# shaofeifei11/SSDR-AL

Hardware: AMD Instinct MI355X
Metric: Mpoints/s subsample→KNN→RandLA-Net→FPS-GCN select, S3DIS 40960-pt tiles (higher is better)
Workload: dtype bf16x3: split-bf16 MFMA operands (hi*hi + lo*hi + hi*lo), fp32 accumulate, fp32 activations and non-matrix arithmetic

## Files before the change

### ssdr-al_amd/csrc/block_prims.hpp

```cpp
#pragma once
#include "ssdr_internal.hpp"
#include <cfloat>

namespace ssdr {

constexpr int BS = 256;
constexpr int U = 4;
constexpr int CHUNK = BS * U;

#ifndef HIPEMU
template <class Op>
__device__ __forceinline__ unsigned wave_reduce_u32(unsigned x, Op op) {
    x = op(x, (unsigned)__builtin_amdgcn_update_dpp((int)x, (int)x, 0xB1, 0xf, 0xf, true));
    x = op(x, (unsigned)__builtin_amdgcn_update_dpp((int)x, (int)x, 0x4E, 0xf, 0xf, true));
    x = op(x, (unsigned)__builtin_amdgcn_update_dpp((int)x, (int)x, 0x141, 0xf, 0xf, true));
    x = op(x, (unsigned)__builtin_amdgcn_update_dpp((int)x, (int)x, 0x140, 0xf, 0xf, true));
    auto r = __builtin_amdgcn_permlane16_swap(x, x, false, false);
    x = op(r[0], r[1]);
    r = __builtin_amdgcn_permlane32_swap(x, x, false, false);
    return op(r[0], r[1]);
}
__device__ __forceinline__ float wave_min(float v) {
    return __uint_as_float(wave_reduce_u32(__float_as_uint(v), [](unsigned a, unsigned b) { return __float_as_uint(fminf(__uint_as_float(a), __uint_as_float(b))); }));
}
// ... 28 lines not shown
        const int lin = tile * gx + bx, xcd = lin & 7, j = lin >> 3;
        tile = xcd + 8 * (j / gx); bx = j % gx;
    }
}

__device__ __forceinline__ void wave_sync() {
#ifndef HIPEMU
    __builtin_amdgcn_fence(__ATOMIC_RELEASE, "workgroup");
    __builtin_amdgcn_wave_barrier();
    __builtin_amdgcn_fence(__ATOMIC_ACQUIRE, "workgroup");
#else
    (void)__shfl(0, 0);
#endif
}

template <int NT = BS>
__device__ inline void block_minmax3(float (&mn)[3], float (&mx)[3], float* s ) {
    const int lane = threadIdx.x & 63, wid = threadIdx.x >> 6;
#pragma unroll
    for (int d = 0; d < 3; ++d) {
        float a = wave_min(mn[d]), b = wave_max(mx[d]);
        if (lane == 0) { s[wid * 6 + d] = a; s[wid * 6 + 3 + d] = b; }
    }
    __syncthreads();
#pragma unroll
    for (int d = 0; d < 3; ++d) {
        float a = s[d], b = s[3 + d];
#pragma unroll
        for (int w = 1; w < NT / 64; ++w) { a = fminf(a, s[w * 6 + d]); b = fmaxf(b, s[w * 6 + 3 + d]); }
        mn[d] = a; mx[d] = b;
// ... 49 lines not shown
```

### ssdr-al_amd/csrc/frontend.hip

```cpp
#include "ssdr_internal.hpp"
#include "block_prims.hpp"
#include "voxel_label.hpp"
#include "subsample_types.hpp"

namespace ssdr {
namespace {

constexpr int FE_NBMAX = 16384;
constexpr int FE_CH = 32768;
constexpr int FE_NT = 1024;
constexpr int FE_PPT = 12, FE_SNT = 1024;
#ifndef FE_PAIR_STORES
#define FE_PAIR_STORES 1
#endif
constexpr int FE_LR = 64;
constexpr int FE_VMAX = 1024;
#ifndef FE_RNT_OPT
#define FE_RNT_OPT 128
#endif
constexpr int FE_RNT = FE_RNT_OPT;
#ifndef FE_WALK_OPT
#define FE_WALK_OPT 4
#endif
constexpr int FE_WALK = FE_WALK_OPT;
constexpr int FE_CAP = 1024;
constexpr int FE_RPT = FE_CAP / FE_RNT;
constexpr int FE_SLICES = 62;
constexpr int FE_ROWCAP = FE_LR * FE_NBMAX;

struct FeGeom {
    float org[3]; float dl;
    int nx, ny, nz, sx;
    int nbx, nby, nbz, nb;
    int ok, n, pad0, pad1;
};
struct FeItem { unsigned base, n, rb, sx; float org[3]; float dl; };

struct FeTab { int nr; int chunks_max; int ovf_cap; int n_total; int off[RADIX_MAX_SEG + 1]; };

__device__ __forceinline__ bool fe_voxel(const FeGeom& g, float x, float y, float z, int& ix, int& iy, int& iz) {
    const float fx = floorf((x - g.org[0]) / g.dl), fy = floorf((y - g.org[1]) / g.dl), fz = floorf((z - g.org[2]) / g.dl);
    const bool ok = fx >= 0.f && fx < (float)g.nx && fy >= 0.f && fy < (float)g.ny && fz >= 0.f && fz < (float)g.nz;
    ix = (int)fx; iy = (int)fy; iz = (int)fz;
    return ok;
}
__device__ __forceinline__ int fe_bucket(const FeGeom& g, int ix, int iy, int iz) { return (ix >> g.sx) + g.nbx * ((iy >> 3) + g.nby * (iz >> 3)); }
__device__ __forceinline__ int fe_vid(const FeItem& it, float x, float y, float z) {
    const int ix = (int)floorf((x - it.org[0]) / it.dl), iy = (int)floorf((y - it.org[1]) / it.dl), iz = (int)floorf((z - it.org[2]) / it.dl);
    return (ix & ((1 << it.sx) - 1)) | (((iy & 7) | ((iz & 7) << 3)) << it.sx);
}

__global__ __launch_bounds__(BS) void fe_minmax_partial(FeTab t, const float* __restrict__ P, float* partial) {
    const int r = blockIdx.y;
    gs_minmax_partial_body(P + 3 * (size_t)t.off[r], t.off[r + 1] - t.off[r], partial + (size_t)r * PB * 6);
}

__global__ void fe_rcp_init(float* rcp) { const int k = blockIdx.x * blockDim.x + threadIdx.x; if (k <= FE_CAP) rcp[k] = k ? (float)(1.0 / (double)k) : 0.f; }

__global__ __launch_bounds__(BS) void fe_params(FeTab t, const float* partial, float dl, GsParams* prm, FeGeom* geom, int* counters) {
    __shared__ float s_mm[(BS / 64) * 6];
    const int r = blockIdx.x;
    float mn[3] = {FLT_MAX, FLT_MAX, FLT_MAX}, mx[3] = {-FLT_MAX, -FLT_MAX, -FLT_MAX};
    for (int i = threadIdx.x; i < PB; i += BS) {
#pragma unroll
        for (int d = 0; d < 3; ++d) { mn[d] = fminf(mn[d], partial[((size_t)r * PB + i) * 6 + d]); mx[d] = fmaxf(mx[d], partial[((size_t)r * PB + i) * 6 + 3 + d]); }
    }
    block_minmax3(mn, mx, s_mm);
    if (threadIdx.x == 0) {
        if (r == 0) { for (int i = 0; i < 8; ++i) counters[i] = 0; }
        GsParams p; FeGeom g;
        const float inv = 1 / dl;
        float nd[3];
#pragma unroll
        for (int d = 0; d < 3; ++d) { g.org[d] = floorf(mn[d] * inv) * dl; p.org[d] = g.org[d]; nd[d] = floorf((mx[d] - g.org[d]) / dl) + 1.f; }
        g.dl = dl; p.dl = dl;
        bool ok = nd[0] >= 1.f && nd[1] >= 1.f && nd[2] >= 1.f && nd[0] < 65536.f && nd[1] < 1.0e6f && nd[2] < 1.0e6f;
#pragma unroll
        for (int d = 0; d < 3; ++d) ok = ok && floorf((mn[d] - g.org[d]) / dl) >= 0.f;
        g.nx = ok ? (int)nd[0] : 1; g.ny = ok ? (int)nd[1] : 1; g.nz = ok ? (int)nd[2] : 1;
        p.nx = (unsigned long long)g.nx; p.ny = (unsigned long long)g.ny; p.m = 0; p.status = 0; p.key_and = 0ull; p.key_or = ~0ull;
        g.nby = (g.ny + 7) >> 3; g.nbz = (g.nz + 7) >> 3;
        g.sx = 3; g.nbx = (g.nx + 7) >> 3;
        if ((long long)g.nbx * g.nby * g.nbz > FE_NBMAX) { g.sx = 4; g.nbx = (g.nx + 15) >> 4; }
        if ((long long)g.nbx * g.nby * g.nbz > FE_NBMAX) ok = false;
        g.nb = ok ? g.nbx * g.nby * g.nbz : 0;
        g.ok = ok ? 1 : 0; g.n = t.off[r + 1] - t.off[r]; g.pad0 = g.pad1 = 0;
        if (!ok) p.status = 2;
        prm[r] = p; geom[r] = g;
    }
}

__global__ __launch_bounds__(FE_NT) void fe_count(FeTab t, const float* __restrict__ P, const FeGeom* __restrict__ geom, GsParams* prm, unsigned* cntm) {
    __shared__ unsigned s_h[FE_NBMAX];
    const int r = blockIdx.y, c = blockIdx.x, tid = threadIdx.x;
    const FeGeom g = geom[r];
    if (!g.ok || c * FE_CH >= g.n) return;
    for (int b = tid; b < g.nb; b += FE_NT) s_h[b] = 0u;
    __syncthreads();
    const float* Pr = P + 3 * (size_t)t.off[r];
    const int hi = min(g.n, (c + 1) * FE_CH);
    bool bad = false;
    for (int i = c * FE_CH + tid; i < hi; i += FE_NT) {
        int ix, iy, iz;
        if (fe_voxel(g, Pr[3 * (size_t)i], Pr[3 * (size_t)i + 1], Pr[3 * (size_t)i + 2], ix, iy, iz)) atomicAdd(&s_h[fe_bucket(g, ix, iy, iz)], 1u);
// ... 7 lines not shown

__device__ __forceinline__ unsigned long long fe_block_scan(unsigned long long v, unsigned long long* s_w, int nt, unsigned long long& total) {
    const int tid = threadIdx.x, lane = tid & 63, wid = tid >> 6;
    unsigned long long incl = v;
#pragma unroll
    for (int o = 1; o < 64; o <<= 1) { const unsigned long long y = __shfl_up(incl, o); if (lane >= o) incl += y; }
    if (lane == 63) s_w[wid] = incl;
    __syncthreads();
    unsigned long long wbase = 0, tot = 0;
    for (int w = 0; w < nt / 64; ++w) { const unsigned long long cw = s_w[w]; if (w < wid) wbase += cw; tot += cw; }
    __syncthreads();
    total = tot;
    return wbase + incl - v;
}

__global__ __launch_bounds__(BS) void fe_colscan(FeTab t, const FeGeom* __restrict__ geom, unsigned* cntm, unsigned* tot) {
    const int r = blockIdx.y, b = blockIdx.x * BS + threadIdx.x;
    const FeGeom g = geom[r];
    if (!g.ok || b >= g.nb) return;
    const int nchunk = (g.n + FE_CH - 1) / FE_CH;
    unsigned* cm = cntm + (size_t)r * t.chunks_max * FE_NBMAX + b;
    unsigned run = 0;
    for (int c0 = 0; c0 < nchunk; c0 += 8) {
        unsigned v[8];
#pragma unroll
        for (int u = 0; u < 8; ++u) v[u] = c0 + u < nchunk ? cm[(size_t)(c0 + u) * FE_NBMAX] : 0u;
#pragma unroll
        for (int u = 0; u < 8; ++u) if (c0 + u < nchunk) { cm[(size_t)(c0 + u) * FE_NBMAX] = run; run += v[u]; }
    }
    tot[(size_t)r * FE_NBMAX + b] = run;
}

__global__ __launch_bounds__(FE_NT) void fe_bscan(FeTab t, const FeGeom* __restrict__ geom, const unsigned* __restrict__ tot, unsigned* boff, FeItem* items, int* counters) {
    __shared__ unsigned long long s_w[FE_NT / 64];
    __shared__ unsigned s_base;
    const int r = blockIdx.x, tid = threadIdx.x;
    const FeGeom g = geom[r];
    unsigned* bo = boff + (size_t)r * (FE_NBMAX + 1);
    if (!g.ok) { if (tid == 0) bo[0] = 0u; return; }
    unsigned long long carry = 0;
    for (int b0 = 0; b0 < g.nb; b0 += FE_NT) {
        const int b = b0 + tid;
        const unsigned n = b < g.nb ? tot[(size_t)r * FE_NBMAX + b] : 0u;
        unsigned long long total;
        const unsigned long long ex = fe_block_scan(((unsigned long long)n << 20) | (n ? 1ull : 0ull), s_w, FE_NT, total);
        const unsigned start = (unsigned)((carry + ex) >> 20);
        if (b < g.nb) bo[b] = start;
        const unsigned nne = (unsigned)(total & 0xfffffull);
        if (tid == 0) s_base = nne ? (unsigned)atomicAdd(&counters[0], (int)nne) : 0u;
        __syncthreads();
        if (n) {
            FeItem it; it.base = (unsigned)t.off[r] + start; it.n = n; it.rb = ((unsigned)r << 16) | (unsigned)b; it.sx = (unsigned)g.sx;
            it.org[0] = g.org[0]; it.org[1] = g.org[1]; it.org[2] = g.org[2]; it.dl = g.dl;
            items[s_base + (unsigned)(ex & 0xfffffull)] = it;
        }
        carry += total & ~0xfffffull;
        __syncthreads();
    }
// ... 342 lines not shown
                FE_STAMP(2);
                if (ns > 0) fe_reduce_voxels<FD, LD, IMG>(L, a, &prm->status, L.orank[v0], L.orank[v1], s0, rows, R);
                FE_STAMP(3);
            }
            if (tid == 0) { a.nocc[tb] = (unsigned)nocc; a.trow[tb] = (fast && IMG) ? it.base : 0x80000000u | L.ovf; }
            for (int l = tid; l < FE_LR; l += FE_RNT) a.lrc[tb * FE_LR + l] = (unsigned char)(L.orank[(l + 1) << it.sx] - L.orank[l << it.sx]);
        }
        __syncthreads();
        FE_STAMP(4);
    }
#ifdef SSDR_FE_STAMPS
    if (tid == 0) for (int k = 0; k < 5; ++k) atomicAdd(reinterpret_cast<unsigned long long*>(a.counters) + 8 + k, t_acc[k]);
#endif
}

__global__ __launch_bounds__(BS) void fe_rowpre(const FeGeom* __restrict__ geom, const unsigned* __restrict__ boff, const unsigned char* __restrict__ lrc,
                                                unsigned short* pre, unsigned* rowcnt) {
    const int r = blockIdx.y;
    const FeGeom g = geom[r];
    if (!g.ok) return;
    const int ry = g.nby * 8, prows = ry * g.nbz * 8;
    const unsigned* bo = boff + (size_t)r * (FE_NBMAX + 1);
    for (int pr = blockIdx.x * BS + threadIdx.x; pr < prows; pr += gridDim.x * BS) {
        const int iy = pr % ry, iz = pr / ry;
        const int l = (iy & 7) | ((iz & 7) << 3);
        const int b0 = g.nbx * ((iy >> 3) + g.nby * (iz >> 3));
        unsigned run = 0;
        for (int bx = 0; bx < g.nbx; ++bx) {
            const int b = b0 + bx;
            if (bo[b + 1] != bo[b]) {
                const size_t at = ((size_t)r * FE_NBMAX + b) * FE_LR + l;
                pre[at] = (unsigned short)run;
                run += lrc[at];
            }
        }
        rowcnt[(size_t)r * FE_ROWCAP + pr] = run;
    }
}

__global__ __launch_bounds__(FE_NT) void fe_rowscan(const FeGeom* __restrict__ geom, unsigned* rowcnt, GsParams* prm, long long* out_m) {
    __shared__ unsigned long long s_w[FE_NT / 64];
    const int r = blockIdx.x, tid = threadIdx.x;
    const FeGeom g = geom[r];
    if (!g.ok) { if (tid == 0) { prm[r].m = 0; if (out_m) out_m[r] = 0; } return; }
    const int prows = g.nby * 8 * g.nbz * 8;
    unsigned* rc = rowcnt + (size_t)r * FE_ROWCAP;
    unsigned long long carry = 0;
    for (int p0 = 0; p0 < prows; p0 += FE_NT) {
        const int p = p0 + tid;
        const unsigned v = p < prows ? rc[p] : 0u;
        unsigned long long total;
        const unsigned long long ex = fe_block_scan((unsigned long long)v, s_w, FE_NT, total);
        if (p < prows) rc[p] = (unsigned)(carry + ex);
        carry += total;
    }
    if (tid == 0) { prm[r].m = (int)carry; if (out_m) out_m[r] = (long long)carry; }
}

struct FeMoveArgs {
    FeTab t; const FeGeom* geom; const FeItem* items; const int* counters; const uint4* rec; const unsigned* nocc; const unsigned* trow;
    const unsigned char* lrc; const unsigned short* pre; const unsigned* rowbase; int fdim, ldim; float* out_p; float* out_f; int* out_c;
};
template <int FD, int LD>
__global__ __launch_bounds__(BS) void fe_move(FeMoveArgs a) {
    const int fdim = FD >= 0 ? FD : a.fdim, ldim = LD >= 0 ? LD : a.ldim;
// ... 58 lines not shown
    FeTab t; t.nr = (int)nr;
    int maxn = 0;
    for (size_t r = 0; r < nr; ++r) {
        const long n = (long)(room_off[r + 1] - room_off[r]);
        if (n <= 0 || room_off[r + 1] > 0x3fffffff) { set_error("grid_subsample_batch: every cloud needs >= 1 point"); return n <= 0 ? SSDR_ERR_EMPTY : SSDR_ERR_INVALID; }
        t.off[r] = (int)room_off[r]; maxn = std::max(maxn, (int)n);
    }
    t.off[nr] = (int)room_off[nr];
    t.n_total = (int)room_off[nr];
    t.chunks_max = (maxn + FE_CH - 1) / FE_CH;
    static const bool fe_image = [] { const char* e = getenv("SSDR_FE_IMAGE"); return e && e[0] == '1'; }();
    static const int fe_wgs = [] { const char* e = getenv("SSDR_FE_WGS"); return e ? atoi(e) : 0; }();
    static const int fe_pad = [] { const char* e = getenv("SSDR_FE_PADLDS"); return e ? atoi(e) : 0; }();
    t.ovf_cap = fe_image ? std::max(65536, t.n_total / 8) : t.n_total;
    const unsigned R = (unsigned)nr;
    SSDR_TRY(S.partial.reserve(24 * (size_t)PB * nr)); SSDR_TRY(S.geom.reserve(sizeof(FeGeom) * nr)); SSDR_TRY(S.counters.reserve(256));
    SSDR_TRY(S.cntm.reserve(4 * (size_t)FE_NBMAX * t.chunks_max * nr)); SSDR_TRY(S.tot.reserve(4 * (size_t)FE_NBMAX * nr)); SSDR_TRY(S.boff.reserve(4 * (size_t)(FE_NBMAX + 1) * nr));
    SSDR_TRY(S.items.reserve(sizeof(FeItem) * (size_t)FE_NBMAX * nr)); SSDR_TRY(S.nocc.reserve(4 * (size_t)FE_NBMAX * nr)); SSDR_TRY(S.trow.reserve(4 * (size_t)FE_NBMAX * nr));
    SSDR_TRY(S.lrc.reserve((size_t)FE_NBMAX * FE_LR * nr)); SSDR_TRY(S.pre.reserve(2 * (size_t)FE_NBMAX * FE_LR * nr));
    SSDR_TRY(S.rowcnt.reserve(4 * (size_t)FE_ROWCAP * nr));
    SSDR_TRY(S.rec.reserve(32 * ((size_t)t.n_total + t.ovf_cap) + 64));
    if (!S.rcp_ready) {
        SSDR_TRY(S.rcp.reserve(4 * (FE_CAP + 1)));
        hipLaunchKernelGGL(fe_rcp_init, dim3((FE_CAP + 256) / 256), dim3(256), 0, s, S.rcp.as<float>());
        S.rcp_ready = true;
    }
    FeGeom* geom = S.geom.as<FeGeom>(); int* counters = S.counters.as<int>(); FeItem* items = S.items.as<FeItem>();
    {
    ProfScope prof("fe_bbox_count_scan", s, 0.0);
    hipLaunchKernelGGL(fe_minmax_partial, dim3(PB, R), dim3(BS), 0, s, t, d_p, S.partial.as<float>());
    hipLaunchKernelGGL(fe_params, dim3(R), dim3(BS), 0, s, t, S.partial.as<float>(), dl, prm, geom, counters);
    hipLaunchKernelGGL(fe_count, dim3(t.chunks_max, R), dim3(FE_NT), 0, s, t, d_p, geom, prm, S.cntm.as<unsigned>());
    hipLaunchKernelGGL(fe_colscan, dim3(FE_NBMAX / BS, R), dim3(BS), 0, s, t, geom, S.cntm.as<unsigned>(), S.tot.as<unsigned>());
    hipLaunchKernelGGL(fe_bscan, dim3(R), dim3(FE_NT), 0, s, t, geom, S.tot.as<unsigned>(), S.boff.as<unsigned>(), items, counters);
    }
    {
    ProfScope prof("fe_scatter", s, (double)(12 + 4 * (fdim + ldim)) * (double)t.n_total);
    if (fdim == 3 && ldim == 1)
        hipLaunchKernelGGL((fe_scatter<3, 1>), dim3(t.chunks_max, R), dim3(FE_SNT), 0, s, t, d_p, d_f, (int)fdim, (const int*)d_c, (int)ldim, geom, S.cntm.as<unsigned>(), S.boff.as<unsigned>(),
                           S.rec.as<uint4>());
    else
        hipLaunchKernelGGL((fe_scatter<-1, -1>), dim3(t.chunks_max, R), dim3(FE_SNT), 0, s, t, d_p, d_f, (int)fdim, (const int*)d_c, (int)ldim, geom, S.cntm.as<unsigned>(), S.boff.as<unsigned>(),
                           S.rec.as<uint4>());
    }
    FeRedArgs ra; ra.t = t; ra.items = items; ra.prm = prm; ra.counters = counters; ra.rcp = S.rcp.as<float>(); ra.rec = S.rec.as<uint4>();
    ra.nocc = S.nocc.as<unsigned>(); ra.trow = S.trow.as<unsigned>(); ra.lrc = S.lrc.as<unsigned char>(); ra.fdim = (int)fdim; ra.ldim = (int)ldim;
    {
    ProfScope prof("fe_reduce", s, 0.0);
    if (!fe_image) {
        const long cap = std::max<long>((long)ctx().num_cu * 16, (long)t.n_total / 64);
        const int g = (int)std::min<long>((long)ctx().num_cu * (fe_wgs > 0 ? fe_wgs : 128), fe_wgs > 0 ? (1L << 30) : cap);
        if (fdim == 3 && ldim == 1) hipLaunchKernelGGL((fe_reduce<3, 1, false>), dim3(g), dim3(FE_RNT), (size_t)fe_pad, s, ra);
        else hipLaunchKernelGGL((fe_reduce<-1, -1, false>), dim3(g), dim3(FE_RNT), (size_t)fe_pad, s, ra);
    } else if (fdim == 3 && ldim == 1) hipLaunchKernelGGL((fe_reduce<3, 1, true>), dim3(ctx().num_cu * (fe_wgs > 0 ? fe_wgs : 3)), dim3(FE_RNT), 0, s, ra);
    else hipLaunchKernelGGL((fe_reduce<-1, -1, true>), dim3(ctx().num_cu * (fe_wgs > 0 ? fe_wgs : 3)), dim3(FE_RNT), 0, s, ra);
    }
    ProfScope prof_move("fe_rows_move", s, 0.0);
    hipLaunchKernelGGL(fe_rowpre, dim3(256, R), dim3(BS), 0, s, geom, S.boff.as<unsigned>(), S.lrc.as<unsigned char>(), S.pre.as<unsigned short>(), S.rowcnt.as<unsigned>());
    hipLaunchKernelGGL(fe_rowscan, dim3(R), dim3(FE_NT), 0, s, geom, S.rowcnt.as<unsigned>(), prm, (long long*)d_om);
    FeMoveArgs ma; ma.t = t; ma.geom = geom; ma.items = items; ma.counters = counters; ma.rec = S.rec.as<uint4>(); ma.nocc = S.nocc.as<unsigned>();
    ma.trow = S.trow.as<unsigned>(); ma.lrc = S.lrc.as<unsigned char>(); ma.pre = S.pre.as<unsigned short>(); ma.rowbase = S.rowcnt.as<unsigned>(); ma.fdim = (int)fdim; ma.ldim = (int)ldim;
    ma.out_p = d_op; ma.out_f = d_of; ma.out_c = d_oc;
    static const int mv_wgs = [] { const char* e = getenv("SSDR_FE_MOVE_WGS"); return e ? atoi(e) : 32; }();
    if (fdim == 3 && ldim == 1) hipLaunchKernelGGL((fe_move<3, 1>), dim3(ctx().num_cu * mv_wgs), dim3(BS), 0, s, ma);
    else hipLaunchKernelGGL((fe_move<-1, -1>), dim3(ctx().num_cu * mv_wgs), dim3(BS), 0, s, ma);
    SSDR_HIP(hipGetLastError());
#ifdef SSDR_FE_STAMPS
    {
        SSDR_HIP(hipStreamSynchronize(s));
        unsigned long long h[8]; int hc[8];
        SSDR_HIP(hipMemcpy(hc, counters, sizeof(hc), hipMemcpyDeviceToHost));
        SSDR_HIP(hipMemcpy(h, reinterpret_cast<unsigned long long*>(counters) + 8, sizeof(h), hipMemcpyDeviceToHost));
        fprintf(stderr, "fe_reduce: %d items, %d overflow rows; clock ticks per phase (sum over workgroups): load+hist %llu, segments %llu, rank %llu, voxels %llu, tail %llu\n",
                hc[0], hc[3], h[0], h[1], h[2], h[3], h[4]);
// ... 8 lines not shown
```

### ssdr-al_amd/csrc/tile.hip

```cpp
#include "ssdr_internal.hpp"
#include "block_prims.hpp"
#include "tile_body.hpp"
#include <map>
#include <vector>

namespace ssdr {
namespace {

__device__ __forceinline__ void tile_keys_body(const float* __restrict__ pts, const long long* __restrict__ d_m, int n_host, float cx, float cy, float cz,
                                                 uint64_t* keys, uint32_t* vals, int* d_count) {
    const int m = (int)min((long long)n_host, *d_m);
    if (blockIdx.x == 0 && threadIdx.x == 0) *d_count = m;
    for (int i = blockIdx.x * 256 + threadIdx.x; i < m; i += gridDim.x * 256) {
        const float dx = pts[3 * (size_t)i] - cx, dy = pts[3 * (size_t)i + 1] - cy, dz = pts[3 * (size_t)i + 2] - cz;
        const float d = (dx * dx + dy * dy) + dz * dz;
        if (vals) { keys[i] = (uint64_t)__float_as_uint(d); vals[i] = (uint32_t)i; }
        else keys[i] = ((uint64_t)__float_as_uint(d) << 32) | (uint64_t)(uint32_t)i;
    }
}


__global__ __launch_bounds__(256) void tile_keys(const float* __restrict__ pts, const long long* __restrict__ d_m, int n_host, float cx, float cy, float cz, uint64_t* keys, uint32_t* vals, int* d_count) { tile_keys_body(pts, d_m, n_host, cx, cy, cz, keys, vals, d_count); }
__global__ __launch_bounds__(256) void tile_padmap(const int* __restrict__ d_count, int num_points, const int* __restrict__ perm, int* padmap) { __shared__ unsigned s_part[256]; tile_padmap_body(*d_count, num_points, perm, padmap, s_part); }
__global__ __launch_bounds__(256) void tile_gather(const float* __restrict__ pts, const float* __restrict__ colors, int cdim, const uint32_t* __restrict__ sorted, const int* __restrict__ d_count, const int* __restrict__ perm, const float* __restrict__ dup_u, int num_points, float cx, float cy, float cz, float color_scale, float* out_xyz, float* out_feat, int* out_idx, const int* __restrict__ padmap) { tile_gather_body(pts, colors, cdim, sorted, d_count, perm, dup_u, num_points, cx, cy, cz, color_scale, out_xyz, out_feat, out_idx, padmap); }
// ... 5 lines not shown
    tile_keys_body(pts + 3 * (size_t)t.off[r], d_m + r, t.off[r + 1] - t.off[r], t.cx[r], t.cy[r], t.cz[r], keys + t.toff[r], vals ? vals + t.toff[r] : nullptr, d_count + r);
}
__global__ __launch_bounds__(256) void tile_gather_b(TileTab t, const float* __restrict__ pts, const float* __restrict__ colors, int cdim, const uint32_t* __restrict__ sorted,
                                                     const int* __restrict__ d_count, const int* __restrict__ perm, const float* __restrict__ dup_u, int num_points,
                                                     float color_scale, float* out_xyz, float* out_feat, int* out_idx, int stride,
                                                     const int* __restrict__ labels, int* out_lab, const int* __restrict__ padmap) {
    int bx, r; xcd_tile_map(bx, r);
    const size_t o = (size_t)t.off[r], q = (size_t)r * num_points;
    tile_gather_body(pts + 3 * o, colors ? colors + o * cdim : nullptr, cdim, sorted + (size_t)t.toff[r] * stride, d_count + r, perm + q, dup_u + q, num_points, t.cx[r], t.cy[r], t.cz[r],
                     color_scale, out_xyz + 3 * q, out_feat ? out_feat + q * (3 + cdim) : nullptr, out_idx ? out_idx + q : nullptr, padmap + q, stride, bx,
                     labels ? labels + o : nullptr, out_lab ? out_lab + q : nullptr);
}

constexpr int TS_BITS = 14, TS_BINS = 1 << TS_BITS, TS_SHIFT = 31 - TS_BITS;

__global__ __launch_bounds__(256) void tile_hist_b(TileTab t, const float* __restrict__ pts, const long long* __restrict__ d_m, unsigned* hist, int* d_count) {
    __shared__ unsigned s_h[TS_BINS];
    const int r = blockIdx.y, n_host = t.off[r + 1] - t.off[r];
    const int m = (int)min((long long)n_host, d_m[r]);
    if (blockIdx.x == 0 && threadIdx.x == 0) d_count[r] = m;
    if ((int)blockIdx.x * 256 >= m) return;
    for (int b = threadIdx.x; b < TS_BINS; b += 256) s_h[b] = 0u;
    __syncthreads();
    const float* P = pts + 3 * (size_t)t.off[r];
    for (int i = blockIdx.x * 256 + threadIdx.x; i < m; i += gridDim.x * 256)
        atomicAdd(&s_h[__float_as_uint(tile_dist(P, i, t.cx[r], t.cy[r], t.cz[r])) >> TS_SHIFT], 1u);
    __syncthreads();
    for (int b = threadIdx.x; b < TS_BINS; b += 256) if (s_h[b]) atomicAdd(&hist[(size_t)r * TS_BINS + b], s_h[b]);
}
constexpr int TS_RCAP = 4096, TS_RSTEP = 1024;
__global__ __launch_bounds__(256) void tile_thresh_b(TileTab t, unsigned* hist, const int* __restrict__ d_count, int num_points, unsigned* thr, int* d_cand, unsigned* rstart, unsigned* rcur, int rstride,
                                                     const int* __restrict__ perm, int* padmap) {
    __shared__ unsigned s_h[TS_BINS + TS_BINS / 32];
    __shared__ unsigned s_part[256];
    __shared__ unsigned s_T;
    const int r = blockIdx.x, tid = threadIdx.x;
    unsigned* h = hist + (size_t)r * TS_BINS;
    unsigned* RS = rstart + (size_t)r * rstride;
    constexpr int PER = TS_BINS / 256;
    auto at = [](int b) { return b + (b >> 5); };
    const unsigned want = (unsigned)min(num_points, d_count[r]);
    for (int b = tid; b < TS_BINS; b += 256) s_h[at(b)] = h[b];
    for (int k = tid; k < rstride; k += 256) { RS[k] = 0xffffffffu; rcur[(size_t)r * rstride + k] = 0u; }
    __syncthreads();
    unsigned tot = 0;
    for (int k = 0; k < PER; ++k) tot += s_h[at(tid * PER + k)];
    s_part[tid] = tot;
    __syncthreads();
    unsigned incl = tot;
    for (int o = 1; o < 256; o <<= 1) {
        const unsigned y = tid >= o ? s_part[tid - o] : 0u;
        __syncthreads();
        incl += y; s_part[tid] = incl;
        __syncthreads();
    }
    const unsigned before = incl - tot;
    if (want > 0 && before < want && incl >= want) {
// ... 5 lines not shown
    __syncthreads();
    const unsigned T = s_T;
    unsigned pos = before, ncand = 0;
    for (int k = 0; k < PER; ++k) {
        const int b = tid * PER + k;
        const unsigned cb = s_h[at(b)];
        if ((unsigned)b <= T) {
            s_h[at(b)] = pos;
            if (cb) atomicMin(&RS[pos / TS_RSTEP], pos);
            pos += cb; ncand = pos;
        } else s_h[at(b)] = 0u;
    }
    if ((unsigned)(tid * PER) <= T && (unsigned)(tid * PER + PER - 1) >= T) { thr[r] = T; d_cand[r] = (int)ncand; }
    __syncthreads();
    for (int b = tid; b < TS_BINS; b += 256) h[b] = s_h[at(b)];
    tile_padmap_body(d_count[r], num_points, perm + (size_t)r * num_points, padmap + (size_t)r * num_points, s_part);
}
constexpr int TS_CPT = 12;
constexpr int TS_RMAX = 2048;
__global__ __launch_bounds__(256) void tile_compact_b(TileTab t, const float* __restrict__ pts, const int* __restrict__ d_count, const unsigned* __restrict__ thr,
                                                      const unsigned* __restrict__ hist, const unsigned* __restrict__ rstart, unsigned* rcur, int rstride, uint64_t* keys) {
    __shared__ unsigned s_cnt[TS_RMAX], s_base[TS_RMAX];
    const int r = blockIdx.y, m = d_count[r], tid = threadIdx.x;
    const float* P = pts + 3 * (size_t)t.off[r];
    const unsigned T = thr[r];
    const unsigned* h = hist + (size_t)r * TS_BINS;
    const unsigned* RS = rstart + (size_t)r * rstride;
    unsigned* RC = rcur + (size_t)r * rstride;
    uint64_t* K = keys + t.toff[r];
    for (int i0 = blockIdx.x * 256 * TS_CPT; i0 < m; i0 += gridDim.x * 256 * TS_CPT) {
        for (int k = tid; k < rstride; k += 256) s_cnt[k] = 0u;
// ... 18 lines not shown
        __syncthreads();
    }
}
__global__ __launch_bounds__(256) void tile_compact_bins_b(TileTab t, const float* __restrict__ pts, const int* __restrict__ d_count, const unsigned* __restrict__ thr, unsigned* hist, uint64_t* keys) {
    const int r = blockIdx.y, m = d_count[r];
    const float* P = pts + 3 * (size_t)t.off[r];
    const unsigned T = thr[r];
    unsigned* cur = hist + (size_t)r * TS_BINS;
    uint64_t* K = keys + t.toff[r];
    for (int i = blockIdx.x * 256 + threadIdx.x; i < m; i += gridDim.x * 256) {
        const unsigned bits = __float_as_uint(tile_dist(P, i, t.cx[r], t.cy[r], t.cz[r]));
        const unsigned b = bits >> TS_SHIFT;
        if (b <= T) K[atomicAdd(&cur[b], 1u)] = ((uint64_t)bits << 32) | (uint64_t)(uint32_t)i;
    }
}
__global__ __launch_bounds__(256) void tile_clear_b(unsigned* hist) {
    for (int b = blockIdx.x * 256 + threadIdx.x; b < TS_BINS; b += gridDim.x * 256) hist[(size_t)blockIdx.y * TS_BINS + b] = 0u;
}
__global__ __launch_bounds__(256) void tile_binsort_b(TileTab t, const unsigned* __restrict__ rstart, int rstride, const int* __restrict__ d_cand, uint64_t* keys) {
    __shared__ uint64_t s_k[TS_RCAP];
    const int r = blockIdx.y, tid = threadIdx.x;
    const unsigned* RS = rstart + (size_t)r * rstride;
    uint64_t* K = keys + t.toff[r];
    const unsigned cand = (unsigned)d_cand[r];
    const int nk = (int)((cand + TS_RSTEP - 1) / TS_RSTEP);
    for (int q = blockIdx.x; q < nk; q += gridDim.x) {
        const unsigned s0 = RS[q];
        if (s0 == 0xffffffffu) continue;
        unsigned e0 = cand;
        for (int q2 = q + 1; q2 < nk; ++q2) if (RS[q2] != 0xffffffffu) { e0 = RS[q2]; break; }
        const unsigned n = e0 - s0;
        if (n <= 1) continue;
        unsigned N = 2; while (N < n) N <<= 1;
        const bool lds = n <= (unsigned)TS_RCAP;
        uint64_t* A = lds ? s_k : K + s0;
        if (N <= 2048u && N >= 16u) {
// ... 139 lines not shown
    if (d_out_feat && color_dim > 0 && !d_colors) { set_error("tile_select_batch: colors missing"); return SSDR_ERR_INVALID; }
    SSDR_TRY(ensure_init());
    hipStream_t s = pick_stream(stream); TileState& T = tst(s);
    TileTab t; t.nr = (int)num_clouds;
    int toff = 0, maxn = 0; std::vector<int> n_host(num_clouds);
    for (size_t r = 0; r < num_clouds; ++r) {
        const long n = (long)(cloud_offsets[r + 1] - cloud_offsets[r]);
        if (n <= 0 || cloud_offsets[r + 1] > 0x3fffffff) { set_error("tile_select_batch: bad cloud offsets"); return SSDR_ERR_INVALID; }
        t.off[r] = (int)cloud_offsets[r]; t.toff[r] = toff; n_host[r] = (int)n; maxn = std::max(maxn, (int)n);
        t.cx[r] = centers[3 * r]; t.cy[r] = centers[3 * r + 1]; t.cz[r] = centers[3 * r + 2];
        toff += ((int)n + RADIX_TILE - 1) / RADIX_TILE * RADIX_TILE;
    }
    t.off[num_clouds] = (int)cloud_offsets[num_clouds]; t.toff[num_clouds] = toff;
    SSDR_TRY(T.keys.reserve(8 * (size_t)toff + 16)); SSDR_TRY(T.count.reserve(4 * num_clouds + 16));
    const int rstride = (maxn + TS_RSTEP - 1) / TS_RSTEP + 1;
    SSDR_TRY(T.hist.reserve(4 * (size_t)TS_BINS * RADIX_MAX_SEG)); SSDR_TRY(T.thr.reserve(4 * RADIX_MAX_SEG)); SSDR_TRY(T.cand.reserve(4 * RADIX_MAX_SEG));
    SSDR_TRY(T.rstart.reserve(4 * (size_t)rstride * num_clouds)); SSDR_TRY(T.rcur.reserve(4 * (size_t)rstride * num_clouds));
    SSDR_TRY(T.padmap.reserve(4 * num_clouds * num_points));
    if (!T.hist_clear) { SSDR_HIP(hipMemsetAsync(T.hist.p, 0, 4 * (size_t)TS_BINS * RADIX_MAX_SEG, s)); T.hist_clear = true; }
    const unsigned R = (unsigned)num_clouds;
    const int g = std::max(1, std::min((maxn + 255) / 256, 64));
    ProfScope prof("tile_select", s, (12.0 + 4.0 * (12 + 4 * (d_out_feat ? color_dim + 3 : 0))) * 0.0 + 40.0 * (double)num_clouds * (double)num_points);
    hipLaunchKernelGGL(tile_hist_b, dim3(g, R), dim3(256), 0, s, t, d_points, (const long long*)d_m, T.hist.as<unsigned>(), T.count.as<int>());
    hipLaunchKernelGGL(tile_thresh_b, dim3(R), dim3(256), 0, s, t, T.hist.as<unsigned>(), T.count.as<int>(), (int)num_points, T.thr.as<unsigned>(), T.cand.as<int>(), T.rstart.as<unsigned>(), T.rcur.as<unsigned>(), rstride,
                       d_perm, T.padmap.as<int>());
    if (rstride <= TS_RMAX)
        hipLaunchKernelGGL(tile_compact_b, dim3(std::max(1, std::min((maxn + 256 * TS_CPT - 1) / (256 * TS_CPT), 256)), R), dim3(256), 0, s, t, d_points, T.count.as<int>(), T.thr.as<unsigned>(),
                           T.hist.as<unsigned>(), T.rstart.as<unsigned>(), T.rcur.as<unsigned>(), rstride, T.keys.as<uint64_t>());
    else hipLaunchKernelGGL(tile_compact_bins_b, dim3(g, R), dim3(256), 0, s, t, d_points, T.count.as<int>(), T.thr.as<unsigned>(), T.hist.as<unsigned>(), T.keys.as<uint64_t>());
    hipLaunchKernelGGL(tile_clear_b, dim3(8, R), dim3(256), 0, s, T.hist.as<unsigned>());
    hipLaunchKernelGGL(tile_binsort_b, dim3(std::min(rstride, 64), R), dim3(256), 0, s, t, T.rstart.as<unsigned>(), rstride, T.cand.as<int>(), T.keys.as<uint64_t>());
    const int g2 = (int)std::max<size_t>(1, std::min<size_t>((num_points + 255) / 256, 256));
    hipLaunchKernelGGL(tile_gather_b, dim3(g2, R), dim3(256), 0, s, t, d_points, d_colors, d_colors ? color_dim : 0, reinterpret_cast<const uint32_t*>(T.keys.as<uint64_t>()), T.count.as<int>(),
                       d_perm, d_dup_u, (int)num_points, color_scale, d_out_xyz, d_out_feat, d_out_idx, 2, d_labels, d_out_labels, T.padmap.as<int>());
    SSDR_HIP(hipGetLastError());
    return SSDR_OK;
}
```

Before: 205.1.

## Fuse dependent frontend and tile-select kernel pairs via last-workgroup tickets

Merges several producer/consumer kernel pairs (minmax→params, colscan→bscan, rowpre→rowscan, hist→thresh) into single launches. The last workgroup to finish, detected with a per-cloud atomic ticket counter, runs the serial tail. The histogram clear is folded into binsort. This removes kernel launches and inter-kernel gaps in small, latency-bound stages. In exchange it adds atomic tickets and fences, and the tail now runs in only one workgroup, with changed block sizes for colscan and rowpre. The tickets reset themselves, so correctness depends on every workgroup reaching the ticket.

After: 155.7. -24.1%, worse.

```diff
diff --git a/ssdr-al_amd/csrc/block_prims.hpp b/ssdr-al_amd/csrc/block_prims.hpp
--- a/ssdr-al_amd/csrc/block_prims.hpp
+++ b/ssdr-al_amd/csrc/block_prims.hpp
@@ -66,6 +66,29 @@
 #endif
 }
 
+template <class T>
+__device__ __forceinline__ T dev_load(const T* p) {
+#ifndef HIPEMU
+    return __hip_atomic_load(p, __ATOMIC_RELAXED, __HIP_MEMORY_SCOPE_AGENT);
+#else
+    T v; __atomic_load(p, &v, __ATOMIC_RELAXED); return v;
+#endif
+}
+__device__ __forceinline__ bool last_workgroup(int* ticket, int expected) {
+    __shared__ int s_last;
+    __threadfence();
+    __syncthreads();
+    if (threadIdx.x == 0) {
+        const int last = atomicAdd(ticket, 1) == expected - 1 ? 1 : 0;
+        if (last) atomicExch(ticket, 0);
+        s_last = last;
+    }
+    __syncthreads();
+    const bool last = s_last != 0;
+    if (last) __threadfence();
+    return last;
+}
+
 template <int NT = BS>
 __device__ inline void block_minmax3(float (&mn)[3], float (&mx)[3], float* s ) {
     const int lane = threadIdx.x & 63, wid = threadIdx.x >> 6;
diff --git a/ssdr-al_amd/csrc/frontend.hip b/ssdr-al_amd/csrc/frontend.hip
--- a/ssdr-al_amd/csrc/frontend.hip
+++ b/ssdr-al_amd/csrc/frontend.hip
@@ -27,6 +27,7 @@
 constexpr int FE_RPT = FE_CAP / FE_RNT;
 constexpr int FE_SLICES = 62;
 constexpr int FE_ROWCAP = FE_LR * FE_NBMAX;
+constexpr size_t FE_COUNTER_BYTES = 256 + 3 * 4 * (size_t)RADIX_MAX_SEG;
 
 struct FeGeom {
     float org[3]; float dl;
@@ -50,24 +51,16 @@
     return (ix & ((1 << it.sx) - 1)) | (((iy & 7) | ((iz & 7) << 3)) << it.sx);
 }
 
-__global__ __launch_bounds__(BS) void fe_minmax_partial(FeTab t, const float* __restrict__ P, float* partial) {
-    const int r = blockIdx.y;
-    gs_minmax_partial_body(P + 3 * (size_t)t.off[r], t.off[r + 1] - t.off[r], partial + (size_t)r * PB * 6);
-}
-
 __global__ void fe_rcp_init(float* rcp) { const int k = blockIdx.x * blockDim.x + threadIdx.x; if (k <= FE_CAP) rcp[k] = k ? (float)(1.0 / (double)k) : 0.f; }
 
-__global__ __launch_bounds__(BS) void fe_params(FeTab t, const float* partial, float dl, GsParams* prm, FeGeom* geom, int* counters) {
-    __shared__ float s_mm[(BS / 64) * 6];
-    const int r = blockIdx.x;
+__device__ __forceinline__ void fe_params_body(const FeTab& t, int r, const float* partial, float dl, GsParams* prm, FeGeom* geom, float* s_mm) {
     float mn[3] = {FLT_MAX, FLT_MAX, FLT_MAX}, mx[3] = {-FLT_MAX, -FLT_MAX, -FLT_MAX};
     for (int i = threadIdx.x; i < PB; i += BS) {
 #pragma unroll
-        for (int d = 0; d < 3; ++d) { mn[d] = fminf(mn[d], partial[((size_t)r * PB + i) * 6 + d]); mx[d] = fmaxf(mx[d], partial[((size_t)r * PB + i) * 6 + 3 + d]); }
+        for (int d = 0; d < 3; ++d) { mn[d] = fminf(mn[d], dev_load(&partial[((size_t)r * PB + i) * 6 + d])); mx[d] = fmaxf(mx[d], dev_load(&partial[((size_t)r * PB + i) * 6 + 3 + d])); }
     }
     block_minmax3(mn, mx, s_mm);
     if (threadIdx.x == 0) {
-        if (r == 0) { for (int i = 0; i < 8; ++i) counters[i] = 0; }
         GsParams p; FeGeom g;
         const float inv = 1 / dl;
         float nd[3];
@@ -88,6 +81,14 @@
         if (!ok) p.status = 2;
         prm[r] = p; geom[r] = g;
     }
+}
+__global__ __launch_bounds__(BS) void fe_minmax_partial_params(FeTab t, const float* __restrict__ P, float* partial, float dl, GsParams* prm, FeGeom* geom, int* counters, int* tickets) {
+    __shared__ float s_mm[(BS / 64) * 6];
+    const int r = blockIdx.y;
+    if (r == 0 && blockIdx.x == 0 && threadIdx.x == 0) { for (int i = 0; i < 8; ++i) counters[i] = 0; }
+    gs_minmax_partial_body(P + 3 * (size_t)t.off[r], t.off[r + 1] - t.off[r], partial + (size_t)r * PB * 6);
+    if (!last_workgroup(tickets + r, PB)) return;
+    fe_params_body(t, r, partial, dl, prm, geom, s_mm);
 }
 
 __global__ __launch_bounds__(FE_NT) void fe_count(FeTab t, const float* __restrict__ P, const FeGeom* __restrict__ geom, GsParams* prm, unsigned* cntm) {
@@ -125,34 +126,35 @@
     return wbase + incl - v;
 }
 
-__global__ __launch_bounds__(BS) void fe_colscan(FeTab t, const FeGeom* __restrict__ geom, unsigned* cntm, unsigned* tot) {
-    const int r = blockIdx.y, b = blockIdx.x * BS + threadIdx.x;
-    const FeGeom g = geom[r];
-    if (!g.ok || b >= g.nb) return;
-    const int nchunk = (g.n + FE_CH - 1) / FE_CH;
-    unsigned* cm = cntm + (size_t)r * t.chunks_max * FE_NBMAX + b;
-    unsigned run = 0;
-    for (int c0 = 0; c0 < nchunk; c0 += 8) {
-        unsigned v[8];
-#pragma unroll
-        for (int u = 0; u < 8; ++u) v[u] = c0 + u < nchunk ? cm[(size_t)(c0 + u) * FE_NBMAX] : 0u;
-#pragma unroll
-        for (int u = 0; u < 8; ++u) if (c0 + u < nchunk) { cm[(size_t)(c0 + u) * FE_NBMAX] = run; run += v[u]; }
-    }
-    tot[(size_t)r * FE_NBMAX + b] = run;
-}
-
-__global__ __launch_bounds__(FE_NT) void fe_bscan(FeTab t, const FeGeom* __restrict__ geom, const unsigned* __restrict__ tot, unsigned* boff, FeItem* items, int* counters) {
+__global__ __launch_bounds__(FE_NT) void fe_colscan_bscan(FeTab t, const FeGeom* __restrict__ geom, unsigned* cntm, unsigned* tot, unsigned* boff, FeItem* items, int* counters, int* tickets) {
     __shared__ unsigned long long s_w[FE_NT / 64];
     __shared__ unsigned s_base;
-    const int r = blockIdx.x, tid = threadIdx.x;
+    const int r = blockIdx.y, tid = threadIdx.x;
     const FeGeom g = geom[r];
     unsigned* bo = boff + (size_t)r * (FE_NBMAX + 1);
-    if (!g.ok) { if (tid == 0) bo[0] = 0u; return; }
+    if (!g.ok) { if (blockIdx.x == 0 && tid == 0) bo[0] = 0u; return; }
+    if ((int)blockIdx.x * FE_NT >= g.nb) return;
+    {
+        const int b = blockIdx.x * FE_NT + tid;
+        if (b < g.nb) {
+            const int nchunk = (g.n + FE_CH - 1) / FE_CH;
+            unsigned* cm = cntm + (size_t)r * t.chunks_max * FE_NBMAX + b;
+            unsigned run = 0;
+            for (int c0 = 0; c0 < nchunk; c0 += 8) {
+                unsigned v[8];
+#pragma unroll
+                for (int u = 0; u < 8; ++u) v[u] = c0 + u < nchunk ? cm[(size_t)(c0 + u) * FE_NBMAX] : 0u;
+#pragma unroll
+                for (int u = 0; u < 8; ++u) if (c0 + u < nchunk) { cm[(size_t)(c0 + u) * FE_NBMAX] = run; run += v[u]; }
+            }
+            tot[(size_t)r * FE_NBMAX + b] = run;
+        }
+    }
+    if (!last_workgroup(tickets + r, (g.nb + FE_NT - 1) / FE_NT)) return;
     unsigned long long carry = 0;
     for (int b0 = 0; b0 < g.nb; b0 += FE_NT) {
         const int b = b0 + tid;
-        const unsigned n = b < g.nb ? tot[(size_t)r * FE_NBMAX + b] : 0u;
+        const unsigned n = b < g.nb ? dev_load(&tot[(size_t)r * FE_NBMAX + b]) : 0u;
         unsigned long long total;
         const unsigned long long ex = fe_block_scan(((unsigned long long)n << 20) | (n ? 1ull : 0ull), s_w, FE_NT, total);
         const unsigned start = (unsigned)((carry + ex) >> 20);
@@ -525,14 +527,17 @@
 #endif
 }
 
-__global__ __launch_bounds__(BS) void fe_rowpre(const FeGeom* __restrict__ geom, const unsigned* __restrict__ boff, const unsigned char* __restrict__ lrc,
-                                                unsigned short* pre, unsigned* rowcnt) {
-    const int r = blockIdx.y;
+__global__ __launch_bounds__(FE_NT) void fe_rowpre_scan(const FeGeom* __restrict__ geom, const unsigned* __restrict__ boff, const unsigned char* __restrict__ lrc,
+                                                        unsigned short* pre, unsigned* rowcnt, GsParams* prm, long long* out_m, int* tickets) {
+    __shared__ unsigned long long s_w[FE_NT / 64];
+    const int r = blockIdx.y, tid = threadIdx.x;
     const FeGeom g = geom[r];
-    if (!g.ok) return;
+    if (!g.ok) { if (blockIdx.x == 0 && tid == 0) { prm[r].m = 0; if (out_m) out_m[r] = 0; } return; }
     const int ry = g.nby * 8, prows = ry * g.nbz * 8;
+    if ((int)blockIdx.x * FE_NT >= prows) return;
     const unsigned* bo = boff + (size_t)r * (FE_NBMAX + 1);
-    for (int pr = blockIdx.x * BS + threadIdx.x; pr < prows; pr += gridDim.x * BS) {
+    unsigned* rc = rowcnt + (size_t)r * FE_ROWCAP;
+    for (int pr = blockIdx.x * FE_NT + tid; pr < prows; pr += gridDim.x * FE_NT) {
         const int iy = pr % ry, iz = pr / ry;
         const int l = (iy & 7) | ((iz & 7) << 3);
         const int b0 = g.nbx * ((iy >> 3) + g.nby * (iz >> 3));
@@ -545,21 +550,13 @@
                 run += lrc[at];
             }
         }
-        rowcnt[(size_t)r * FE_ROWCAP + pr] = run;
-    }
-}
-
-__global__ __launch_bounds__(FE_NT) void fe_rowscan(const FeGeom* __restrict__ geom, unsigned* rowcnt, GsParams* prm, long long* out_m) {
-    __shared__ unsigned long long s_w[FE_NT / 64];
-    const int r = blockIdx.x, tid = threadIdx.x;
-    const FeGeom g = geom[r];
-    if (!g.ok) { if (tid == 0) { prm[r].m = 0; if (out_m) out_m[r] = 0; } return; }
-    const int prows = g.nby * 8 * g.nbz * 8;
-    unsigned* rc = rowcnt + (size_t)r * FE_ROWCAP;
+        rc[pr] = run;
+    }
+    if (!last_workgroup(tickets + r, min((int)gridDim.x, (prows + FE_NT - 1) / FE_NT))) return;
     unsigned long long carry = 0;
     for (int p0 = 0; p0 < prows; p0 += FE_NT) {
         const int p = p0 + tid;
-        const unsigned v = p < prows ? rc[p] : 0u;
+        const unsigned v = p < prows ? dev_load(&rc[p]) : 0u;
         unsigned long long total;
         const unsigned long long ex = fe_block_scan((unsigned long long)v, s_w, FE_NT, total);
         if (p < prows) rc[p] = (unsigned)(carry + ex);
@@ -648,25 +645,26 @@
     static const int fe_pad = [] { const char* e = getenv("SSDR_FE_PADLDS"); return e ? atoi(e) : 0; }();
     t.ovf_cap = fe_image ? std::max(65536, t.n_total / 8) : t.n_total;
     const unsigned R = (unsigned)nr;
-    SSDR_TRY(S.partial.reserve(24 * (size_t)PB * nr)); SSDR_TRY(S.geom.reserve(sizeof(FeGeom) * nr)); SSDR_TRY(S.counters.reserve(256));
+    SSDR_TRY(S.partial.reserve(24 * (size_t)PB * nr)); SSDR_TRY(S.geom.reserve(sizeof(FeGeom) * nr)); SSDR_TRY(S.counters.reserve(FE_COUNTER_BYTES));
     SSDR_TRY(S.cntm.reserve(4 * (size_t)FE_NBMAX * t.chunks_max * nr)); SSDR_TRY(S.tot.reserve(4 * (size_t)FE_NBMAX * nr)); SSDR_TRY(S.boff.reserve(4 * (size_t)(FE_NBMAX + 1) * nr));
     SSDR_TRY(S.items.reserve(sizeof(FeItem) * (size_t)FE_NBMAX * nr)); SSDR_TRY(S.nocc.reserve(4 * (size_t)FE_NBMAX * nr)); SSDR_TRY(S.trow.reserve(4 * (size_t)FE_NBMAX * nr));
     SSDR_TRY(S.lrc.reserve((size_t)FE_NBMAX * FE_LR * nr)); SSDR_TRY(S.pre.reserve(2 * (size_t)FE_NBMAX * FE_LR * nr));
     SSDR_TRY(S.rowcnt.reserve(4 * (size_t)FE_ROWCAP * nr));
     SSDR_TRY(S.rec.reserve(32 * ((size_t)t.n_total + t.ovf_cap) + 64));
     if (!S.rcp_ready) {
+        SSDR_HIP(hipMemsetAsync(S.counters.p, 0, FE_COUNTER_BYTES, s));
         SSDR_TRY(S.rcp.reserve(4 * (FE_CAP + 1)));
         hipLaunchKernelGGL(fe_rcp_init, dim3((FE_CAP + 256) / 256), dim3(256), 0, s, S.rcp.as<float>());
         S.rcp_ready = true;
     }
     FeGeom* geom = S.geom.as<FeGeom>(); int* counters = S.counters.as<int>(); FeItem* items = S.items.as<FeItem>();
+    int* tickets = counters + 64;
     {
     ProfScope prof("fe_bbox_count_scan", s, 0.0);
-    hipLaunchKernelGGL(fe_minmax_partial, dim3(PB, R), dim3(BS), 0, s, t, d_p, S.partial.as<float>());
-    hipLaunchKernelGGL(fe_params, dim3(R), dim3(BS), 0, s, t, S.partial.as<float>(), dl, prm, geom, counters);
+    hipLaunchKernelGGL(fe_minmax_partial_params, dim3(PB, R), dim3(BS), 0, s, t, d_p, S.partial.as<float>(), dl, prm, geom, counters, tickets);
     hipLaunchKernelGGL(fe_count, dim3(t.chunks_max, R), dim3(FE_NT), 0, s, t, d_p, geom, prm, S.cntm.as<unsigned>());
-    hipLaunchKernelGGL(fe_colscan, dim3(FE_NBMAX / BS, R), dim3(BS), 0, s, t, geom, S.cntm.as<unsigned>(), S.tot.as<unsigned>());
-    hipLaunchKernelGGL(fe_bscan, dim3(R), dim3(FE_NT), 0, s, t, geom, S.tot.as<unsigned>(), S.boff.as<unsigned>(), items, counters);
+    hipLaunchKernelGGL(fe_colscan_bscan, dim3(FE_NBMAX / FE_NT, R), dim3(FE_NT), 0, s, t, geom, S.cntm.as<unsigned>(), S.tot.as<unsigned>(), S.boff.as<unsigned>(), items, counters,
+                       tickets + RADIX_MAX_SEG);
     }
     {
     ProfScope prof("fe_scatter", s, (double)(12 + 4 * (fdim + ldim)) * (double)t.n_total);
@@ -690,8 +688,8 @@
     else hipLaunchKernelGGL((fe_reduce<-1, -1, true>), dim3(ctx().num_cu * (fe_wgs > 0 ? fe_wgs : 3)), dim3(FE_RNT), 0, s, ra);
     }
     ProfScope prof_move("fe_rows_move", s, 0.0);
-    hipLaunchKernelGGL(fe_rowpre, dim3(256, R), dim3(BS), 0, s, geom, S.boff.as<unsigned>(), S.lrc.as<unsigned char>(), S.pre.as<unsigned short>(), S.rowcnt.as<unsigned>());
-    hipLaunchKernelGGL(fe_rowscan, dim3(R), dim3(FE_NT), 0, s, geom, S.rowcnt.as<unsigned>(), prm, (long long*)d_om);
+    hipLaunchKernelGGL(fe_rowpre_scan, dim3(64, R), dim3(FE_NT), 0, s, geom, S.boff.as<unsigned>(), S.lrc.as<unsigned char>(), S.pre.as<unsigned short>(), S.rowcnt.as<unsigned>(), prm,
+                       (long long*)d_om, tickets + 2 * RADIX_MAX_SEG);
     FeMoveArgs ma; ma.t = t; ma.geom = geom; ma.items = items; ma.counters = counters; ma.rec = S.rec.as<uint4>(); ma.nocc = S.nocc.as<unsigned>();
     ma.trow = S.trow.as<unsigned>(); ma.lrc = S.lrc.as<unsigned char>(); ma.pre = S.pre.as<unsigned short>(); ma.rowbase = S.rowcnt.as<unsigned>(); ma.fdim = (int)fdim; ma.ldim = (int)ldim;
     ma.out_p = d_op; ma.out_f = d_of; ma.out_c = d_oc;
diff --git a/ssdr-al_amd/csrc/tile.hip b/ssdr-al_amd/csrc/tile.hip
--- a/ssdr-al_amd/csrc/tile.hip
+++ b/ssdr-al_amd/csrc/tile.hip
@@ -43,33 +43,31 @@
 
 constexpr int TS_BITS = 14, TS_BINS = 1 << TS_BITS, TS_SHIFT = 31 - TS_BITS;
 
-__global__ __launch_bounds__(256) void tile_hist_b(TileTab t, const float* __restrict__ pts, const long long* __restrict__ d_m, unsigned* hist, int* d_count) {
-    __shared__ unsigned s_h[TS_BINS];
-    const int r = blockIdx.y, n_host = t.off[r + 1] - t.off[r];
-    const int m = (int)min((long long)n_host, d_m[r]);
-    if (blockIdx.x == 0 && threadIdx.x == 0) d_count[r] = m;
-    if ((int)blockIdx.x * 256 >= m) return;
-    for (int b = threadIdx.x; b < TS_BINS; b += 256) s_h[b] = 0u;
-    __syncthreads();
-    const float* P = pts + 3 * (size_t)t.off[r];
-    for (int i = blockIdx.x * 256 + threadIdx.x; i < m; i += gridDim.x * 256)
-        atomicAdd(&s_h[__float_as_uint(tile_dist(P, i, t.cx[r], t.cy[r], t.cz[r])) >> TS_SHIFT], 1u);
-    __syncthreads();
-    for (int b = threadIdx.x; b < TS_BINS; b += 256) if (s_h[b]) atomicAdd(&hist[(size_t)r * TS_BINS + b], s_h[b]);
-}
 constexpr int TS_RCAP = 4096, TS_RSTEP = 1024;
-__global__ __launch_bounds__(256) void tile_thresh_b(TileTab t, unsigned* hist, const int* __restrict__ d_count, int num_points, unsigned* thr, int* d_cand, unsigned* rstart, unsigned* rcur, int rstride,
-                                                     const int* __restrict__ perm, int* padmap) {
+__global__ __launch_bounds__(256) void tile_hist_thresh_b(TileTab t, const float* __restrict__ pts, const long long* __restrict__ d_m, unsigned* hist, int* d_count, int num_points, unsigned* thr, int* d_cand,
+                                                          unsigned* rstart, unsigned* rcur, int rstride, const int* __restrict__ perm, int* padmap, int* tickets) {
     __shared__ unsigned s_h[TS_BINS + TS_BINS / 32];
     __shared__ unsigned s_part[256];
     __shared__ unsigned s_T;
-    const int r = blockIdx.x, tid = threadIdx.x;
+    const int r = blockIdx.y, tid = threadIdx.x, n_host = t.off[r + 1] - t.off[r];
+    const int m = (int)min((long long)n_host, d_m[r]);
     unsigned* h = hist + (size_t)r * TS_BINS;
+    if (blockIdx.x == 0 && tid == 0) d_count[r] = m;
+    if ((int)blockIdx.x * 256 < m) {
+        for (int b = tid; b < TS_BINS; b += 256) s_h[b] = 0u;
+        __syncthreads();
+        const float* P = pts + 3 * (size_t)t.off[r];
+        for (int i = blockIdx.x * 256 + tid; i < m; i += gridDim.x * 256)
+            atomicAdd(&s_h[__float_as_uint(tile_dist(P, i, t.cx[r], t.cy[r], t.cz[r])) >> TS_SHIFT], 1u);
+        __syncthreads();
+        for (int b = tid; b < TS_BINS; b += 256) if (s_h[b]) atomicAdd(&h[b], s_h[b]);
+    }
+    if (!last_workgroup(tickets + r, (int)gridDim.x)) return;
     unsigned* RS = rstart + (size_t)r * rstride;
     constexpr int PER = TS_BINS / 256;
     auto at = [](int b) { return b + (b >> 5); };
-    const unsigned want = (unsigned)min(num_points, d_count[r]);
-    for (int b = tid; b < TS_BINS; b += 256) s_h[at(b)] = h[b];
+    const unsigned want = (unsigned)min(num_points, m);
+    for (int b = tid; b < TS_BINS; b += 256) s_h[at(b)] = dev_load(&h[b]);
     for (int k = tid; k < rstride; k += 256) { RS[k] = 0xffffffffu; rcur[(size_t)r * rstride + k] = 0u; }
     __syncthreads();
     unsigned tot = 0;
@@ -105,7 +103,7 @@
     if ((unsigned)(tid * PER) <= T && (unsigned)(tid * PER + PER - 1) >= T) { thr[r] = T; d_cand[r] = (int)ncand; }
     __syncthreads();
     for (int b = tid; b < TS_BINS; b += 256) h[b] = s_h[at(b)];
-    tile_padmap_body(d_count[r], num_points, perm + (size_t)r * num_points, padmap + (size_t)r * num_points, s_part);
+    tile_padmap_body(m, num_points, perm + (size_t)r * num_points, padmap + (size_t)r * num_points, s_part);
 }
 constexpr int TS_CPT = 12;
 constexpr int TS_RMAX = 2048;
@@ -154,12 +152,10 @@
         if (b <= T) K[atomicAdd(&cur[b], 1u)] = ((uint64_t)bits << 32) | (uint64_t)(uint32_t)i;
     }
 }
-__global__ __launch_bounds__(256) void tile_clear_b(unsigned* hist) {
-    for (int b = blockIdx.x * 256 + threadIdx.x; b < TS_BINS; b += gridDim.x * 256) hist[(size_t)blockIdx.y * TS_BINS + b] = 0u;
-}
-__global__ __launch_bounds__(256) void tile_binsort_b(TileTab t, const unsigned* __restrict__ rstart, int rstride, const int* __restrict__ d_cand, uint64_t* keys) {
+__global__ __launch_bounds__(256) void tile_binsort_b(TileTab t, const unsigned* __restrict__ rstart, int rstride, const int* __restrict__ d_cand, uint64_t* keys, unsigned* hist) {
     __shared__ uint64_t s_k[TS_RCAP];
     const int r = blockIdx.y, tid = threadIdx.x;
+    for (int b = blockIdx.x * 256 + tid; b < TS_BINS; b += gridDim.x * 256) hist[(size_t)r * TS_BINS + b] = 0u;
     const unsigned* RS = rstart + (size_t)r * rstride;
     uint64_t* K = keys + t.toff[r];
     const unsigned cand = (unsigned)d_cand[r];
@@ -329,22 +325,23 @@
     t.off[num_clouds] = (int)cloud_offsets[num_clouds]; t.toff[num_clouds] = toff;
     SSDR_TRY(T.keys.reserve(8 * (size_t)toff + 16)); SSDR_TRY(T.count.reserve(4 * num_clouds + 16));
     const int rstride = (maxn + TS_RSTEP - 1) / TS_RSTEP + 1;
-    SSDR_TRY(T.hist.reserve(4 * (size_t)TS_BINS * RADIX_MAX_SEG)); SSDR_TRY(T.thr.reserve(4 * RADIX_MAX_SEG)); SSDR_TRY(T.cand.reserve(4 * RADIX_MAX_SEG));
+    const size_t hist_bytes = 4 * (size_t)TS_BINS * RADIX_MAX_SEG;
+    SSDR_TRY(T.hist.reserve(hist_bytes + 4 * RADIX_MAX_SEG)); SSDR_TRY(T.thr.reserve(4 * RADIX_MAX_SEG)); SSDR_TRY(T.cand.reserve(4 * RADIX_MAX_SEG));
     SSDR_TRY(T.rstart.reserve(4 * (size_t)rstride * num_clouds)); SSDR_TRY(T.rcur.reserve(4 * (size_t)rstride * num_clouds));
     SSDR_TRY(T.padmap.reserve(4 * num_clouds * num_points));
-    if (!T.hist_clear) { SSDR_HIP(hipMemsetAsync(T.hist.p, 0, 4 * (size_t)TS_BINS * RADIX_MAX_SEG, s)); T.hist_clear = true; }
+    if (!T.hist_clear) { SSDR_HIP(hipMemsetAsync(T.hist.p, 0, hist_bytes + 4 * RADIX_MAX_SEG, s)); T.hist_clear = true; }
+    int* tickets = reinterpret_cast<int*>(T.hist.as<unsigned char>() + hist_bytes);
     const unsigned R = (unsigned)num_clouds;
     const int g = std::max(1, std::min((maxn + 255) / 256, 64));
     ProfScope prof("tile_select", s, (12.0 + 4.0 * (12 + 4 * (d_out_feat ? color_dim + 3 : 0))) * 0.0 + 40.0 * (double)num_clouds * (double)num_points);
-    hipLaunchKernelGGL(tile_hist_b, dim3(g, R), dim3(256), 0, s, t, d_points, (const long long*)d_m, T.hist.as<unsigned>(), T.count.as<int>());
-    hipLaunchKernelGGL(tile_thresh_b, dim3(R), dim3(256), 0, s, t, T.hist.as<unsigned>(), T.count.as<int>(), (int)num_points, T.thr.as<unsigned>(), T.cand.as<int>(), T.rstart.as<unsigned>(), T.rcur.as<unsigned>(), rstride,
-                       d_perm, T.padmap.as<int>());
+    hipLaunchKernelGGL(tile_hist_thresh_b, dim3(g, R), dim3(256), 0, s, t, d_points, (const long long*)d_m, T.hist.as<unsigned>(), T.count.as<int>(), (int)num_points, T.thr.as<unsigned>(), T.cand.as<int>(),
+                       T.rstart.as<unsigned>(), T.rcur.as<unsigned>(), rstride, d_perm, T.padmap.as<int>(), tickets);
     if (rstride <= TS_RMAX)
         hipLaunchKernelGGL(tile_compact_b, dim3(std::max(1, std::min((maxn + 256 * TS_CPT - 1) / (256 * TS_CPT), 256)), R), dim3(256), 0, s, t, d_points, T.count.as<int>(), T.thr.as<unsigned>(),
                            T.hist.as<unsigned>(), T.rstart.as<unsigned>(), T.rcur.as<unsigned>(), rstride, T.keys.as<uint64_t>());
     else hipLaunchKernelGGL(tile_compact_bins_b, dim3(g, R), dim3(256), 0, s, t, d_points, T.count.as<int>(), T.thr.as<unsigned>(), T.hist.as<unsigned>(), T.keys.as<uint64_t>());
-    hipLaunchKernelGGL(tile_clear_b, dim3(8, R), dim3(256), 0, s, T.hist.as<unsigned>());
-    hipLaunchKernelGGL(tile_binsort_b, dim3(std::min(rstride, 64), R), dim3(256), 0, s, t, T.rstart.as<unsigned>(), rstride, T.cand.as<int>(), T.keys.as<uint64_t>());
+    hipLaunchKernelGGL(tile_binsort_b, dim3(std::min(rstride, 64), R), dim3(256), 0, s, t, T.rstart.as<unsigned>(), rstride, T.cand.as<int>(), T.keys.as<uint64_t>(),
+                       T.hist.as<unsigned>());
     const int g2 = (int)std::max<size_t>(1, std::min<size_t>((num_points + 255) / 256, 256));
     hipLaunchKernelGGL(tile_gather_b, dim3(g2, R), dim3(256), 0, s, t, d_points, d_colors, d_colors ? color_dim : 0, reinterpret_cast<const uint32_t*>(T.keys.as<uint64_t>()), T.count.as<int>(),
                        d_perm, d_dup_u, (int)num_points, color_scale, d_out_xyz, d_out_feat, d_out_idx, 2, d_labels, d_out_labels, T.padmap.as<int>());
```
